# ucas-vg/PointTinyBenchmark

Measured on NVIDIA H100. Metric: cpr_head_refine_img_per_s_1333x800, higher is better.
Workload: dtype fp32

## Files before the change

include/ptb_b200.h:

```cpp
#ifndef PTB_B200_H_
#define PTB_B200_H_

#include <stdint.h>

#ifdef __cplusplus
extern "C" {
#endif

#define PTB_ABI_VERSION 1

int ptb_abi_version(void);
const char* ptb_last_error(void);
uint64_t ptb_launch_count(void);
int ptb_reset_stream_state(void* stream);

int ptb_cpr_bag_gather(const float* map, int B, int H, int W, int C, int ld,
                       const float* centers , const int32_t* bag_img , int G,
                       const float* offsets , int K, float stride,
                       float reach_px ,
                       const int32_t* pad_hw ,
                       float* out_feats , float* out_pts , uint8_t* out_valid ,
                       void* stream);

int ptb_cpr_bag_gather_bwd(const float* grad_out , int B, int H, int W, int C, int ld,
// ... 217 lines not shown
                            int B, int H, int W, int Cin, float* y , double* gn_stats, void* stream);
int ptb_gn_relu_apply(const float* y, const double* gn_stats, const float* gamma, const float* beta, int B, int HW, int C,
                      int groups, float eps, int relu, float* out_hi, float* out_lo, void* stream);
int ptb_split_f16(const float* x, int64_t n, int auto_scale, void* hi, void* lo, float* dev_inv_scale, void* workspace, void* stream);
int ptb_conv3x3_pack_weight_f16(const float* w_oihw, int Cout, int Cin, float scale, void* w_h, void* w_l, void* stream);
int ptb_conv3x3_c256_f16x2(const void* x_h, const void* x_l, const void* w_h, const void* w_l, int B, int H, int W, int Cin,
                           float out_scale, const float* dev_out_scale, float* y, double* gn_stats, void* stream);
int ptb_conv_tc_pack_weight_f16(const float* w , int n_out, int n_mma, int Cin, int taps, float scale,
                                void* w_h, void* w_l, void* stream);
int ptb_conv_tc_f16x2(const void* x_h, const void* x_l, const void* w_h, const void* w_l, int B, int H, int W, int Cin, int taps,
                      int n_out, int n_mma, float out_scale, const float* dev_out_scale, const float* bias, float* y, int ldy,
                      void* stream);
int ptb_gn_relu_apply_f16(const float* y, const double* gn_stats, const float* gamma, const float* beta, int B, int HW, int C,
                          int groups, float eps, int relu, void* out_h, void* out_l, int* overflow_flag, void* stream);
#define PTB_DTYPE_F16 1
#define PTB_DTYPE_BF16 2
int ptb_split_f16_from_bf16(const void* x, int64_t n, void* hi, void* lo, float* dev_inv_scale, void* workspace, void* stream);
int ptb_conv_tc_f16x1a(const void* x_h, const void* w_h, const void* w_l, int B, int H, int W, int Cin, int taps, int n_out, int n_mma,
                       float out_scale, const float* dev_out_scale, const float* bias, float* y, int ldy, double* gn_stats ,
                       void* stream);
int ptb_conv_tc_f16x2_half_out(const void* x_h, const void* x_l, const void* w_h, const void* w_l, int B, int H, int W, int Cin, int taps,
                               int n_out, int n_mma, float out_scale, const float* dev_out_scale, const float* bias, void* y, int y_dtype,
                               int ldy, void* stream);

uint64_t ptb_max_iou_assign_workspace(int N, int n_gt);
int ptb_max_iou_assign(const float* bboxes, int N, const float* gt_bboxes, int n_gt, const int32_t* gt_labels ,
                       const float* gt_bboxes_ignore , int n_ignore, float pos_iou_thr, float neg_iou_lo, float neg_iou_hi,
                       float min_pos_iou, int gt_max_assign_all, int match_low_quality, float ignore_iof_thr, int ignore_wrt_candidates,
                       int64_t* out_gt_inds, float* out_max_overlaps, int64_t* out_labels, void* workspace, uint64_t workspace_bytes,
                       void* stream);
int ptb_bbox_overlaps(const float* boxes1, int m, const float* boxes2, int n, int mode_iof, float* out , void* stream);

uint64_t ptb_gn_relu_bwd_workspace(int B, int HW, int C, int groups);
int ptb_gn_relu_bwd(const float* da, const float* y, const double* gn_stats, const float* gamma, const float* beta, int B, int HW, int C,
                    int groups, float eps, int relu, void* workspace, float* dy, float* dgamma ,
                    float* dbeta , unsigned int* amax_bits , void* stream);
int ptb_split_f16_amax(const float* x, int64_t n, const unsigned int* dev_amax_bits, void* hi, void* lo, float* dev_inv_scale,
                       void* stream);
uint64_t ptb_conv3x3_wgrad_workspace(int B, int H, int W);
int ptb_conv3x3_wgrad_f16x2(const void* dy_h, const void* dy_l, const void* x_h, const void* x_l, int B, int H, int W, int Cout, int Cin,
                            float scale, const float* dev_scale_dy , const float* dev_scale_x , void* workspace,
                            float* dw , int accumulate, void* stream);

uint64_t ptb_conv_tc_wgrad_workspace(int B, int H, int W, int taps);
int ptb_conv_tc_wgrad_f16x2(const void* dy_h, const void* dy_l , const void* x_h, const void* x_l ,
                            int B, int H, int W, int Cout, int Cin, int taps, float scale, const float* dev_scale_dy,
// ... 10 lines not shown
```

pointtinybenchmark_b200/_lib.py:

```python
import ctypes
import os

_HERE = os.path.dirname(os.path.abspath(__file__))
LIB_PATH = os.path.join(_HERE, 'libptb_b200.so')

_lib = None
MISSING = []

c_int, c_float, c_void_p, c_u64, c_i64 = ctypes.c_int, ctypes.c_float, ctypes.c_void_p, ctypes.c_uint64, ctypes.c_int64


class RefineCfg(ctypes.Structure):
    _fields_ = [('merge_th', c_float), ('gt_alpha', c_float), ('refine_th', c_float), ('flags', ctypes.c_int32)]


class MatchCost(ctypes.Structure):
    _fields_ = [('kind', ctypes.c_int32), ('weight', c_float), ('alpha', c_float), ('gamma', c_float), ('eps', c_float),
                ('p', ctypes.c_int32), ('norm_with_img_wh', ctypes.c_int32)]


P = c_void_p
SIGNATURES = {
    'ptb_abi_version': (c_int, []),
    'ptb_last_error': (ctypes.c_char_p, []),
# ... 53 lines not shown
    'ptb_hungarian_v2_workspace': (c_u64, [c_int, c_int]),
    'ptb_hungarian_v2_batch': (c_int, [P, P, c_int, c_int, c_int, c_int, P, P, P, P, P]),
    'ptb_point_assigner': (c_int, [P, c_int, P, c_int, c_float, c_int, P, P, c_u64, P]),
    'ptb_point_assigner_workspace': (c_u64, [c_int, c_int]),
    'ptb_sigmoid_focal_fwd_bwd': (c_int, [P, P, P, c_i64, c_int, c_float, c_float, P, P, P, P]),
    'ptb_smooth_l1_fwd_bwd': (c_int, [P, P, P, c_i64, c_float, c_float, P, P, P, P]),
    'ptb_sigmoid_bce_fwd_bwd': (c_int, [P, P, P, c_i64, c_int, P, P, P, P]),
    'ptb_mse_fwd_bwd': (c_int, [P, P, P, c_i64, c_float, P, P, P, P]),
    'ptb_sigmoid_bce_cw_fwd_bwd': (c_int, [P, P, P, P, c_i64, c_int, P, P, P, P]),
    'ptb_softmax_ce_fwd_bwd': (c_int, [P, P, P, P, c_i64, c_int, P, P, P, P]),
    'ptb_split_tf32': (c_int, [P, c_i64, P, P, P]),
    'ptb_conv3x3_pack_weight': (c_int, [P, c_int, c_int, P, P, P]),
    'ptb_conv3x3_c256_tf32x3': (c_int, [P, P, P, P, c_int, c_int, c_int, c_int, P, P, P]),
    'ptb_gn_relu_apply': (c_int, [P, P, P, P, c_int, c_int, c_int, c_int, c_float, c_int, P, P, P]),
    'ptb_split_f16': (c_int, [P, c_i64, c_int, P, P, P, P, P]),
    'ptb_conv3x3_pack_weight_f16': (c_int, [P, c_int, c_int, c_float, P, P, P]),
    'ptb_conv3x3_c256_f16x2': (c_int, [P, P, P, P, c_int, c_int, c_int, c_int, c_float, P, P, P, P]),
    'ptb_conv_tc_pack_weight_f16': (c_int, [P, c_int, c_int, c_int, c_int, c_float, P, P, P]),
    'ptb_conv_tc_f16x2': (c_int, [P, P, P, P, c_int, c_int, c_int, c_int, c_int, c_int, c_int, c_float, P, P, P, c_int, P]),
    'ptb_gn_relu_apply_f16': (c_int, [P, P, P, P, c_int, c_int, c_int, c_int, c_float, c_int, P, P, P, P]),
    'ptb_split_f16_from_bf16': (c_int, [P, c_i64, P, P, P, P, P]),
    'ptb_conv_tc_f16x1a': (c_int, [P, P, P, c_int, c_int, c_int, c_int, c_int, c_int, c_int, c_float, P, P, P, c_int, P, P]),
    'ptb_conv_tc_f16x2_half_out': (c_int, [P, P, P, P, c_int, c_int, c_int, c_int, c_int, c_int, c_int, c_float, P, P, P, c_int, c_int, P]),
    'ptb_max_iou_assign_workspace': (c_u64, [c_int, c_int]),
    'ptb_max_iou_assign': (c_int, [P, c_int, P, c_int, P, P, c_int, c_float, c_float, c_float, c_float, c_int, c_int, c_float, c_int,
                                   P, P, P, P, c_u64, P]),
    'ptb_bbox_overlaps': (c_int, [P, c_int, P, c_int, c_int, P, P]),
    'ptb_gn_relu_bwd_workspace': (c_u64, [c_int, c_int, c_int, c_int]),
    'ptb_gn_relu_bwd': (c_int, [P, P, P, P, P, c_int, c_int, c_int, c_int, c_float, c_int, P, P, P, P, P, P]),
    'ptb_split_f16_amax': (c_int, [P, c_i64, P, P, P, P, P]),
    'ptb_conv3x3_wgrad_workspace': (c_u64, [c_int, c_int, c_int]),
    'ptb_conv3x3_wgrad_f16x2': (c_int, [P, P, P, P, c_int, c_int, c_int, c_int, c_int, c_float, P, P, P, P, c_int, P]),
    'ptb_conv_tc_wgrad_workspace': (c_u64, [c_int, c_int, c_int, c_int]),
    'ptb_conv_tc_wgrad_f16x2': (c_int, [P, P, P, P, c_int, c_int, c_int, c_int, c_int, c_int, c_float, P, P, P, P, c_int, P]),
    'ptb_col_sum_workspace': (c_u64, [c_i64, c_int]),
    'ptb_col_sum': (c_int, [P, c_i64, c_int, c_int, P, P, P]),
}


def load():
    global _lib
    if _lib is not None:
        return _lib
    if not os.path.exists(LIB_PATH):
        raise RuntimeError(
            f'{LIB_PATH} is missing: build it with `python -c "import __graft_entry__ as g; g.build()"` '
# ... 24 lines not shown
```

pointtinybenchmark_b200/csrc/conv_tc.cu:

```cuda
#include "tc_ptx.cuh"
#include <cuda_bf16.h>
#include <stdlib.h>
#include <type_traits>

namespace ptb {

constexpr int CV_N = 256;
constexpr int CV_N_MAX = 512;
constexpr int CV_BM = 128;
constexpr int CV_NT = 128;
constexpr int CV_KB = 16;
constexpr int CV_KB_F16 = 32;
constexpr int CV_KH = 3;
constexpr int CV_A_STAGES = 4;
constexpr int CV_B_STAGES = 8;
constexpr uint32_t CV_A_BYTES = (CV_BM + 2 * 32) * 64;
constexpr uint32_t CV_B_BYTES = CV_NT * 64;
constexpr uint32_t CV_A_STAGE_BYTES = 2 * CV_A_BYTES;
constexpr uint32_t CV_B_STAGE_BYTES = 2 * CV_B_BYTES;
constexpr uint32_t CV_RING_BYTES = CV_A_STAGES * CV_A_STAGE_BYTES + CV_B_STAGES * CV_B_STAGE_BYTES;
constexpr uint32_t CV_SMEM_BYTES = CV_RING_BYTES + 1024  + 256 ;
static_assert(CV_SMEM_BYTES <= 227 * 1024, "the conv rings must fit the 227 KB of opt-in shared memory");
static_assert(2 * 8 * (CV_A_STAGES + CV_B_STAGES) <= 256, "the conv barriers must fit their 256 B");
constexpr int CV_THREADS = 384;

struct ConvShape {
  int B, H, W, Cin;
  int tiles_h, tiles_w;
  int n_main, n_right, n_bottom, per_img, n_tiles;
  int right_w0, right_h;
  int bottom_h0;
  int n_slices;
  int taps;
  int n_out;
  int ldy;
};

struct ConvMaps {
  CUtensorMap x[3][2];
  CUtensorMap w[2];
};
struct TileAt {
  int b, h0, w0, shape, twl;
};
__device__ __forceinline__ TileAt tile_at(const ConvShape& cs, int tile) {
  TileAt t;
  t.b = tile / cs.per_img;
  const int r = tile - t.b * cs.per_img;
  if (r < cs.n_main) {
    t.shape = 0; t.twl = 4; t.h0 = (r / cs.tiles_w) * 8; t.w0 = (r % cs.tiles_w) * 16;
  } else if (r < cs.n_main + cs.n_right) {
    t.shape = 2; t.twl = 3; t.h0 = (r - cs.n_main) * 16; t.w0 = cs.right_w0;
  } else {
    t.shape = 1; t.twl = 5; t.h0 = cs.bottom_h0; t.w0 = (r - cs.n_main - cs.n_right) * 32;
  }
  return t;
}

template <bool F16, int NT, bool A_LO_ZERO = false, typename OutT = float>
__global__ void __launch_bounds__(CV_THREADS, 1)
conv_tc_kernel(const __grid_constant__ ConvMaps mp, ConvShape cs, OutT* __restrict__ y, double* __restrict__ stats ,
               float out_scale, const float* __restrict__ dev_out_scale, const float* __restrict__ bias) {
  static_assert(F16 || NT == 128, "the TF32 mode runs 128-channel slices");
  static_assert(F16 || (!A_LO_ZERO && std::is_same<OutT, float>::value), "half-precision inputs and outputs belong to the fp16 mode");
  constexpr int KBC = F16 ? CV_KB_F16 : CV_KB;
  extern __shared__ uint8_t smem_raw[];
  const uint32_t smem_base = (smem_u32(smem_raw) + 1023u) & ~1023u;
  const uint32_t sA_base = smem_base, sB_base = smem_base + CV_A_STAGES * CV_A_STAGE_BYTES;
  const uint32_t bar_base = smem_base + CV_RING_BYTES;
  auto full_a = [&](int s) { return bar_base + 8u * s; };
  auto empty_a = [&](int s) { return bar_base + 8u * (CV_A_STAGES + s); };
  auto full_b = [&](int s) { return bar_base + 8u * (2 * CV_A_STAGES + s); };
  auto empty_b = [&](int s) { return bar_base + 8u * (2 * CV_A_STAGES + CV_B_STAGES + s); };

  const int wg = threadIdx.x >> 7;
  const int kblocks_per_tap = cs.Cin / KBC;
  const int n_kh = cs.taps == 9 ? CV_KH : 1;
  const int n_boxes_item = (cs.taps / n_kh) * kblocks_per_tap;
  const int n_items = cs.n_tiles * cs.n_slices;

  if (threadIdx.x == 0) {
    for (int s = 0; s < CV_A_STAGES; ++s) {
      mbar_init(full_a(s), 1);
      mbar_init(empty_a(s), 8);
    }
    for (int s = 0; s < CV_B_STAGES; ++s) {
      mbar_init(full_b(s), 1);
      mbar_init(empty_b(s), 8);
    }
    asm volatile("fence.mbarrier_init.release.cluster;" ::: "memory");
  }
  __syncthreads();

  if (wg == 0) {
    regs_dealloc<40>();
    if (threadIdx.x == 0) {
      int a_st = 0, b_st = 0;
      uint32_t a_ph = 0, b_ph = 0;
      for (int item = blockIdx.x; item < n_items; item += gridDim.x) {
        const int tile = item / cs.n_slices, n0 = (item - tile * cs.n_slices) * NT;
        const TileAt ta = tile_at(cs, tile);
        const uint32_t a_bytes = (uint32_t)(CV_BM + ((n_kh - 1) << ta.twl)) * 64u;
        for (int ks = 0; ks < n_boxes_item; ++ks) {
          const int kw = cs.taps == 9 ? ks / kblocks_per_tap : 1, cblk = ks - (ks / kblocks_per_tap) * kblocks_per_tap;
          mbar_wait(empty_a(a_st), a_ph ^ 1u);
          const uint32_t sA_hi = sA_base + a_st * CV_A_STAGE_BYTES;
          mbar_expect_tx(full_a(a_st), (A_LO_ZERO ? 1 : 2) * a_bytes);
          const int aw = ta.w0 + kw - 1, ah = ta.h0 - (n_kh > 1 ? 1 : 0);
          tma_load_4d(&mp.x[ta.shape][0], full_a(a_st), sA_hi, cblk * KBC, aw, ah, ta.b);
          if constexpr (!A_LO_ZERO) tma_load_4d(&mp.x[ta.shape][1], full_a(a_st), sA_hi + CV_A_BYTES, cblk * KBC, aw, ah, ta.b);
          if (++a_st == CV_A_STAGES) { a_st = 0; a_ph ^= 1u; }
          for (int kh = 0; kh < n_kh; ++kh) {
            const int tap = cs.taps == 9 ? 3 * kh + kw : 0;
            const int kcol = tap * cs.Cin + cblk * KBC;
            mbar_wait(empty_b(b_st), b_ph ^ 1u);
            const uint32_t sB_hi = sB_base + b_st * CV_B_STAGE_BYTES;
            mbar_expect_tx(full_b(b_st), 2 * NT * 64);
            tma_load_2d(&mp.w[0], full_b(b_st), sB_hi, kcol, n0);
            tma_load_2d(&mp.w[1], full_b(b_st), sB_hi + CV_B_BYTES, kcol, n0);
            if (++b_st == CV_B_STAGES) { b_st = 0; b_ph ^= 1u; }
          }
        }
      }
    }
  } else {
    regs_alloc<232>();
    const int cw = wg - 1;
    const int t = threadIdx.x & 127, warp = t >> 5, lane = t & 31;
    const float sc = F16 ? (dev_out_scale ? __fmul_rn(out_scale, *dev_out_scale) : out_scale) : 1.f;
    float acc[NT / 2], cor[NT / 2];
    int a_st = 0, b_st = 0;
    uint32_t a_ph = 0, b_ph = 0;
    for (int item = blockIdx.x; item < n_items; item += gridDim.x) {
      const int tile = item / cs.n_slices, n0 = (item - tile * cs.n_slices) * NT;
      const TileAt ta = tile_at(cs, tile);
      const uint32_t kh_step = 64u << ta.twl;
      auto k_loop = [&](auto kh_n_) {
        constexpr int KH_N = decltype(kh_n_)::value;
        int prev_a = 0, prev_b = 0;
        for (int ks = 0; ks < n_boxes_item; ++ks) {
          mbar_wait(full_a(a_st), a_ph);
          const uint32_t sA_hi = sA_base + a_st * CV_A_STAGE_BYTES + (uint32_t)cw * (CV_BM * 64 / 2);
          const uint32_t sA_lo = sA_hi + CV_A_BYTES;
#pragma unroll
          for (int kh = 0; kh < KH_N; ++kh) {
            mbar_wait(full_b(b_st), b_ph);
            const uint32_t a_off = kh_step * kh, sB_hi = sB_base + b_st * CV_B_STAGE_BYTES, sB_lo = sB_hi + CV_B_BYTES;
            wgmma_fence();
#pragma unroll
// ... 75 lines not shown
            ss = fmaf(v0, v0, ss);
            ss = fmaf(v1, v1, ss);
          }
        }
        if constexpr (NT == 128) { part[2 * i] = s; part[2 * i + 1] = ss; }
      }
      if constexpr (NT == 128) {
        if (stats) {
          auto level = [&](auto o_) {
            constexpr int o = decltype(o_)::value;
            const bool up = (lane & o) != 0;
#pragma unroll
            for (int i = 0; i < o; ++i) {
              const float send = up ? part[i] : part[i + o];
              const float recv = __shfl_xor_sync(0xffffffffu, send, o);
              part[i] = (up ? part[i + o] : part[i]) + recv;
            }
          };
          level(std::integral_constant<int, 16>{}); level(std::integral_constant<int, 8>{}); level(std::integral_constant<int, 4>{});
          level(std::integral_constant<int, 2>{}); level(std::integral_constant<int, 1>{});
          atomicAdd(stats + ((size_t)ta.b * 32 + (n0 >> 3) + (lane >> 1)) * 2 + (lane & 1), (double)part[0]);
        }
      }
    }
  }
}

__device__ __forceinline__ float tf32_hi(float x) { return __uint_as_float(__float_as_uint(x) & 0xFFFFE000u); }

__global__ void __launch_bounds__(256)
split_tf32_kernel(const float4* __restrict__ x, long long n4, float4* __restrict__ hi, float4* __restrict__ lo) {
  for (long long i = (long long)blockIdx.x * 256 + threadIdx.x; i < n4; i += (long long)gridDim.x * 256) {
    const float4 v = __ldcs(x + i);
    float4 h = make_float4(tf32_hi(v.x), tf32_hi(v.y), tf32_hi(v.z), tf32_hi(v.w));
    hi[i] = h;
    lo[i] = make_float4(v.x - h.x, v.y - h.y, v.z - h.z, v.w - h.w);
  }
}

__global__ void __launch_bounds__(256)
gn_relu_apply_kernel(const float4* __restrict__ y, const double* __restrict__ stats, const float* __restrict__ gamma,
                     const float* __restrict__ beta, int HW, int C, int groups, float eps, int relu, long long n4,
                     float4* __restrict__ out_hi, float4* __restrict__ out_lo) {
  const int c4n = C >> 2;
  const int cpg = C / groups;
  const double inv_n = 1.0 / ((double)HW * cpg);
// ... 309 lines not shown
  if (n == 0) return 0;
  long long blocks = (n / 4 + 255) / 256;
  const long long cap = (long long)sm_count() * 16;
  if (blocks > cap) blocks = cap;
  split_tf32_kernel<<<(unsigned)blocks, 256, 0, (cudaStream_t)stream>>>(reinterpret_cast<const float4*>(x), n / 4,
                                                                       reinterpret_cast<float4*>(hi), reinterpret_cast<float4*>(lo));
  return check_launch("ptb_split_tf32");
}

extern "C" int ptb_conv3x3_pack_weight(const float* w_oihw, int Cout, int Cin, float* w_hi, float* w_lo, void* stream) {
  PTB_REQUIRE(Cout > 0 && Cin > 0 && w_oihw && w_hi && w_lo, "shape / NULL");
  const long long n = (long long)Cout * Cin * 9;
  pack_conv_weight_kernel<<<(unsigned)((n + 255) / 256), 256, 0, (cudaStream_t)stream>>>(w_oihw, Cout, Cin, w_hi, w_lo);
  return check_launch("ptb_conv3x3_pack_weight");
}

template <bool F16, int NT, bool A_LO_ZERO = false, typename OutT = float>
static int conv_launch_nt(const ConvMaps& mp, const ConvShape& cs, OutT* y, double* gn_stats, float out_scale, const float* dev_out_scale,
                          const float* bias, void* stream) {
  if (cudaFuncSetAttribute(conv_tc_kernel<F16, NT, A_LO_ZERO, OutT>, cudaFuncAttributeMaxDynamicSharedMemorySize, (int)CV_SMEM_BYTES) != cudaSuccess)
    return fail("%s", "cudaFuncSetAttribute(MaxDynamicSharedMemorySize) failed for the conv kernel");
  int grid = sm_count();
  if (grid > cs.n_tiles * cs.n_slices) grid = cs.n_tiles * cs.n_slices;
  conv_tc_kernel<F16, NT, A_LO_ZERO, OutT><<<grid, CV_THREADS, CV_SMEM_BYTES, (cudaStream_t)stream>>>(mp, cs, y, gn_stats, out_scale, dev_out_scale, bias);
  return 0;
}

template <bool F16, bool A_LO_ZERO = false, typename OutT = float>
static int conv_launch(const void* x_hi, const void* x_lo, const void* w_hi, const void* w_lo, int B, int H, int W, int Cin, int taps,
                       int n_out, int n_mma, OutT* y, int ldy, const float* bias, double* gn_stats, float out_scale,
                       const float* dev_out_scale, void* stream, const char* what) {
  ConvShape cs;
  cs.B = B; cs.H = H; cs.W = W; cs.Cin = Cin;
  {
    const int rh = H % 8, rw = W % 16;
    const bool bottom = rh >= 1 && rh <= 4;
    cs.tiles_h = bottom ? H / 8 : (H + 7) / 8;
    cs.bottom_h0 = cs.tiles_h * 8;
    cs.n_bottom = bottom ? (W + 31) / 32 : 0;
    const bool right = rw >= 1 && rw <= 8 && cs.tiles_h > 0;
    cs.tiles_w = right ? W / 16 : (W + 15) / 16;
    cs.right_w0 = cs.tiles_w * 16;
    cs.right_h = cs.tiles_h * 8 < H ? cs.tiles_h * 8 : H;
    cs.n_right = right ? (cs.right_h + 15) / 16 : 0;
    cs.n_main = cs.tiles_h * cs.tiles_w;
    cs.per_img = cs.n_main + cs.n_right + cs.n_bottom;
    cs.n_tiles = B * cs.per_img;
  }
  const int nt = (!F16 || n_mma > 64) ? CV_NT : n_mma > 32 ? 64 : n_mma > 16 ? 32 : 16;
  PTB_REQUIRE(!gn_stats || (n_out == CV_N && n_mma == CV_N && nt == CV_NT), "GroupNorm statistics need 256 output channels (32 groups of 8)");
  cs.n_slices = (n_mma + nt - 1) / nt;
  cs.taps = taps; cs.n_out = n_out; cs.ldy = ldy;
  ConvMaps mp;
  int rc;
  for (int sh = 0; sh < 3; ++sh) {
    if ((rc = make_act_map(&mp.x[sh][0], x_hi, B, H, W, Cin, F16, sh, taps == 9 ? 2 : 0))) return rc;
    if (A_LO_ZERO) mp.x[sh][1] = mp.x[sh][0];
    else if ((rc = make_act_map(&mp.x[sh][1], x_lo, B, H, W, Cin, F16, sh, taps == 9 ? 2 : 0))) return rc;
  }
  if ((rc = make_w_map(&mp.w[0], w_hi, n_mma, taps * Cin, F16, nt))) return rc;
  if ((rc = make_w_map(&mp.w[1], w_lo, n_mma, taps * Cin, F16, nt))) return rc;
  if constexpr (!F16) rc = conv_launch_nt<false, 128>(mp, cs, y, gn_stats, out_scale, dev_out_scale, bias, stream);
  else if (nt == 128) rc = conv_launch_nt<true, 128, A_LO_ZERO, OutT>(mp, cs, y, gn_stats, out_scale, dev_out_scale, bias, stream);
  else if constexpr (!std::is_same<OutT, float>::value) return fail("%s: a half-precision output needs more than 64 output channels", what);
  else if (nt == 64) rc = conv_launch_nt<true, 64, A_LO_ZERO>(mp, cs, y, gn_stats, out_scale, dev_out_scale, bias, stream);
  else if (nt == 32) rc = conv_launch_nt<true, 32, A_LO_ZERO>(mp, cs, y, gn_stats, out_scale, dev_out_scale, bias, stream);
  else rc = conv_launch_nt<true, 16, A_LO_ZERO>(mp, cs, y, gn_stats, out_scale, dev_out_scale, bias, stream);
  if (rc) return rc;
  return check_launch(what);
}

extern "C" int ptb_conv3x3_c256_tf32x3(const float* x_hi, const float* x_lo, const float* w_hi, const float* w_lo, int B, int H,
                                       int W, int Cin, float* y, double* gn_stats, void* stream) {
  PTB_REQUIRE(B > 0 && H > 0 && W > 0 && Cin > 0, "shape");
  PTB_REQUIRE(Cin % CV_KB == 0, "Cin must be a multiple of 16");
  PTB_REQUIRE(x_hi && x_lo && w_hi && w_lo && y, "NULL input");
  PTB_REQUIRE(((uintptr_t)x_hi % 16 == 0) && ((uintptr_t)x_lo % 16 == 0) && ((uintptr_t)w_hi % 16 == 0) &&
                  ((uintptr_t)w_lo % 16 == 0) && ((uintptr_t)y % 16 == 0), "16-byte alignment");
  return conv_launch<false>(x_hi, x_lo, w_hi, w_lo, B, H, W, Cin, 9, CV_N, CV_N, y, CV_N, nullptr, gn_stats, 1.f, nullptr, stream,
                            "ptb_conv3x3_c256_tf32x3");
}

extern "C" int ptb_conv3x3_c256_f16x2(const void* x_h, const void* x_l, const void* w_h, const void* w_l, int B, int H, int W, int Cin,
                                      float out_scale, const float* dev_out_scale, float* y, double* gn_stats, void* stream) {
// ... 75 lines not shown
  PTB_REQUIRE(((uintptr_t)x_h % 16 == 0) && ((uintptr_t)x_l % 16 == 0) && ((uintptr_t)w_h % 16 == 0) && ((uintptr_t)w_l % 16 == 0) &&
                  ((uintptr_t)y % 16 == 0), "16-byte alignment");
  return conv_launch<true>(x_h, x_l, w_h, w_l, B, H, W, Cin, taps, n_out, n_mma, y, ldy, bias, nullptr, out_scale, dev_out_scale, stream,
                           "ptb_conv_tc_f16x2");
}

static int conv_tc_check_shape(int B, int H, int W, int Cin, int taps, int n_out, int n_mma, int ldy) {
  PTB_REQUIRE(B > 0 && H > 0 && W > 0 && Cin > 0 && (taps == 1 || taps == 9), "shape");
  PTB_REQUIRE(Cin % CV_KB_F16 == 0, "Cin must be a multiple of 32");
  PTB_REQUIRE(n_out > 0 && n_mma >= n_out && n_mma % 16 == 0 && n_mma <= CV_N_MAX, "n_mma must be a multiple of 16 in [n_out, 512]");
  PTB_REQUIRE(ldy >= n_out && ldy % 4 == 0, "ldy must be a multiple of 4 and >= n_out");
  return 0;
}

extern "C" int ptb_conv_tc_f16x1a(const void* x_h, const void* w_h, const void* w_l, int B, int H, int W, int Cin, int taps, int n_out,
                                  int n_mma, float out_scale, const float* dev_out_scale, const float* bias, float* y, int ldy,
                                  double* gn_stats, void* stream) {
  if (int rc = conv_tc_check_shape(B, H, W, Cin, taps, n_out, n_mma, ldy)) return rc;
  PTB_REQUIRE(x_h && w_h && w_l && y, "NULL input");
  PTB_REQUIRE(((uintptr_t)x_h % 16 == 0) && ((uintptr_t)w_h % 16 == 0) && ((uintptr_t)w_l % 16 == 0) && ((uintptr_t)y % 16 == 0),
              "16-byte alignment");
  return conv_launch<true, true>(x_h, nullptr, w_h, w_l, B, H, W, Cin, taps, n_out, n_mma, y, ldy, bias, gn_stats, out_scale, dev_out_scale,
                                 stream, "ptb_conv_tc_f16x1a");
}

extern "C" int ptb_conv_tc_f16x2_half_out(const void* x_h, const void* x_l, const void* w_h, const void* w_l, int B, int H, int W, int Cin,
                                          int taps, int n_out, int n_mma, float out_scale, const float* dev_out_scale, const float* bias,
                                          void* y, int y_dtype, int ldy, void* stream) {
  if (int rc = conv_tc_check_shape(B, H, W, Cin, taps, n_out, n_mma, ldy)) return rc;
  PTB_REQUIRE(y_dtype == PTB_DTYPE_F16 || y_dtype == PTB_DTYPE_BF16, "y_dtype must be PTB_DTYPE_F16 or PTB_DTYPE_BF16");
  PTB_REQUIRE(x_h && x_l && w_h && w_l && y, "NULL input");
  PTB_REQUIRE(((uintptr_t)x_h % 16 == 0) && ((uintptr_t)x_l % 16 == 0) && ((uintptr_t)w_h % 16 == 0) && ((uintptr_t)w_l % 16 == 0) &&
                  ((uintptr_t)y % 16 == 0), "16-byte alignment");
  if (y_dtype == PTB_DTYPE_F16)
    return conv_launch<true, false, __half>(x_h, x_l, w_h, w_l, B, H, W, Cin, taps, n_out, n_mma, reinterpret_cast<__half*>(y), ldy, bias,
                                            nullptr, out_scale, dev_out_scale, stream, "ptb_conv_tc_f16x2_half_out");
  return conv_launch<true, false, __nv_bfloat16>(x_h, x_l, w_h, w_l, B, H, W, Cin, taps, n_out, n_mma, reinterpret_cast<__nv_bfloat16*>(y),
                                                 ldy, bias, nullptr, out_scale, dev_out_scale, stream, "ptb_conv_tc_f16x2_half_out");
}

extern "C" int ptb_split_f16_from_bf16(const void* x, int64_t n, void* hi, void* lo, float* dev_inv_scale, void* workspace, void* stream) {
  PTB_REQUIRE(n >= 0 && n % 8 == 0, "n must be a multiple of 8");
  PTB_REQUIRE(((uintptr_t)x % 16 == 0) && ((uintptr_t)hi % 16 == 0) && ((uintptr_t)lo % 16 == 0), "16-byte alignment");
  PTB_REQUIRE(workspace && dev_inv_scale, "a 4-byte workspace and dev_inv_scale are required");
  if (n == 0) return 0;
  cudaStream_t st = (cudaStream_t)stream;
// ... 58 lines not shown
```

pointtinybenchmark_b200/layers.py:

```python
import math

import torch
import torch.nn as nn
import torch.nn.functional as F


class ConvModule(nn.Module):

    def __init__(self, cin, cout, k=3, stride=1, padding=1, norm_cfg=None, bias='auto', act=True):
        super().__init__()
        with_norm = norm_cfg is not None
        if bias == 'auto':
            bias = not with_norm
        self.conv = nn.Conv2d(cin, cout, k, stride, padding, bias=bias)
        self.norm_name = None
        if with_norm:
            t = norm_cfg['type']
            if t == 'GN':
                self.norm_name = 'gn'
                self.add_module('gn', nn.GroupNorm(norm_cfg['num_groups'], cout))
            elif t in ('BN', 'SyncBN'):
                self.norm_name = 'bn'
                self.add_module('bn', nn.BatchNorm2d(cout))
            else:
# ... 140 lines not shown
        c = m.conv
        if not (c.in_channels == 256 and c.out_channels == 256 and c.kernel_size == (3, 3) and c.stride == (1, 1)
                and c.padding == (1, 1) and c.dilation == (1, 1) and c.groups == 1 and c.bias is None and m.norm_name == 'gn'
                and m.with_act and m.gn.num_groups == 32 and m.gn.affine):
            return False
    return True


class _TowerTCFn(torch.autograd.Function):

    @staticmethod
    def forward(ctx, xm, convs, *params):
        from . import ops
        n_layers = len(convs)
        groups, eps = [m.gn.num_groups for m in convs], [float(m.gn.eps) for m in convs]
        h, l, dev_inv = _first_operands(xm)
        half_in = xm.dtype != torch.float32
        flag = torch.zeros(1, dtype=torch.int32, device=xm.device)
        saved, out = [], None
        for i in range(n_layers):
            gamma, beta = params[3 * i + 1], params[3 * i + 2]
            wh, wl, inv_w = _packed_weight_f16(convs[i])
            inv_x = dev_inv if i == 0 else None
            y, stats = ops.conv3x3_c256_f16(h, l, wh, wl, inv_w, inv_x)
            saved += [xm, None, y, stats] if i == 0 and half_in else [h, l, y, stats]
            if i == n_layers - 1:
                out = ops.gn_relu_apply(y, stats, gamma.detach(), beta.detach(), groups[i], eps[i], True, split=False)
            else:
                h, l = ops.gn_relu_apply_f16(y, stats, gamma.detach(), beta.detach(), groups[i], eps[i], True, flag)
        ctx.n_layers, ctx.groups, ctx.eps, ctx.convs = n_layers, groups, eps, convs
        ctx.dev_inv, ctx.in_dtype = dev_inv, xm.dtype
        ctx.save_for_backward(*saved, *[p.detach() for p in params])
        return out

    @staticmethod
    def backward(ctx, dout):
        from . import ops
        n = ctx.n_layers
        saved = ctx.saved_tensors
        acts, params = saved[:4 * n], saved[4 * n:]
        da = dout.contiguous()
        grads = [None] * (3 * n)
        for i in reversed(range(n)):
            h, l, y, stats = acts[4 * i:4 * i + 4]
            inv_x = ctx.dev_inv if i == 0 else None
            if i == 0 and ctx.in_dtype != torch.float32:
                h, l, inv_x = _first_operands(h)
                if l is None:
                    l = torch.zeros_like(h)
            w, gamma, beta = params[3 * i], params[3 * i + 1], params[3 * i + 2]
            dy, dg, db, amax = ops.gn_relu_bwd(da, y, stats, gamma, beta, ctx.groups[i], ctx.eps[i], True)
            dyh, dyl, inv_dy = ops.split_f16_amax(dy, amax)
# ... 4 lines not shown
                da = ops.conv_tc_f16(dyh, dyl, _packed_weight_f16_t(ctx.convs[i]), 9, w.shape[1], dev_out_scale=inv_dy,
                                     out_dtype=ctx.in_dtype if i == 0 else torch.float32)
            else:
                da = None
        return (da, None, *grads)


def tower(convs, x, info=None, want='fp32'):
    import os
    mode = os.environ.get('PTB_CONV_MODE', 'f16x2')
    if x.dtype in HALF_INPUT_DTYPES and not x.is_cuda:
        raise RuntimeError(f'tower: expected a CUDA tensor for a {x.dtype} input (pointtinybenchmark_b200 has no CPU path)')
    plan = input_plan(x.dtype, mode)
    if want == 'f16pair' and not (_tc_supported(convs, x) and mode == 'f16x2' and all(m.conv.in_channels % 32 == 0 for m in convs)):
        return None
    if _tc_supported(convs, x) and mode == 'f16x2' and all(m.conv.in_channels % 32 == 0 for m in convs):
        from . import ops
        xm = ops.to_nhwc(x).contiguous()
        h, l, dev_inv = _first_operands(xm)
        flag = torch.zeros(1, dtype=torch.int32, device=x.device)
        out = None
        for i, m in enumerate(convs):
            wh, wl, inv_w = _packed_weight_f16(m)
            y, stats = ops.conv3x3_c256_f16(h, l, wh, wl, inv_w, dev_inv if i == 0 else None)
            if i == len(convs) - 1 and want == 'fp32':
                out = ops.gn_relu_apply(y, stats, m.gn.weight.detach(), m.gn.bias.detach(), m.gn.num_groups, m.gn.eps, True, split=False)
            else:
                h, l = ops.gn_relu_apply_f16(y, stats, m.gn.weight.detach(), m.gn.bias.detach(), m.gn.num_groups, m.gn.eps, True, flag)
        if info is not None:
            info['backend'] = 'wgmma-f16x2'
            info['input_path'] = plan[0]
            info['overflow_flag'] = flag
        if want == 'f16pair':
            return h, l
        return out.permute(0, 3, 1, 2)
    if _tc_supported(convs, x):
        from . import ops
        xm = ops.to_nhwc(x).contiguous()
        hi, lo = ops.split_tf32(xm)
        out = None
        for i, m in enumerate(convs):
            wh, wl = _packed_weight(m)
            y, stats = ops.conv3x3_c256(hi, lo, wh, wl)
            last = i == len(convs) - 1
            res = ops.gn_relu_apply(y, stats, m.gn.weight.detach(), m.gn.bias.detach(), m.gn.num_groups, m.gn.eps, True,
                                    split=not last)
            if last:
                out = res
            else:
                hi, lo = res
        if info is not None:
# ... 25 lines not shown
```

pointtinybenchmark_b200/ops.py:

```python
import ctypes
import math

import torch

from . import _lib
from ._lib import RefineCfg, check


def _ptr(t):
    return ctypes.c_void_p(t.data_ptr()) if t is not None else ctypes.c_void_p(0)


def _stream():
    return ctypes.c_void_p(torch.cuda.current_stream().cuda_stream)


def _chk(t, dtype, name):
    if not isinstance(t, torch.Tensor) or not t.is_cuda:
        raise RuntimeError(f'{name}: expected a CUDA tensor (pointtinybenchmark_b200 has no CPU path)')
    if t.dtype != dtype:
        raise TypeError(f'{name}: expected {dtype}, got {t.dtype}')
    if not t.is_contiguous():
        raise ValueError(f'{name}: must be contiguous')
    return t
# ... 781 lines not shown
    l = torch.empty_like(h)
    check(lib.ptb_conv3x3_pack_weight_f16(_ptr(w), Cout, Cin, float(scale), _ptr(h), _ptr(l), _stream()), 'ptb_conv3x3_pack_weight_f16')
    return h, l, 1.0 / scale


def conv3x3_c256_f16(x_h, x_l, w_h, w_l, out_scale, dev_out_scale=None, want_stats=True):
    lib = _lib.load()
    _chk(x_h, torch.float16, 'x_h'); _chk(w_h, torch.float16, 'w_h'); _chk(w_l, torch.float16, 'w_l')
    B, H, W, Cin = x_h.shape
    if w_h.shape != (256, 9 * Cin):
        raise ValueError('packed weight must be (256, 9*Cin)')
    y = torch.empty((B, H, W, 256), dtype=torch.float32, device=x_h.device)
    stats = torch.zeros((B, 32, 2), dtype=torch.float64, device=x_h.device) if want_stats else None
    if x_l is None:
        check(lib.ptb_conv_tc_f16x1a(_ptr(x_h), _ptr(w_h), _ptr(w_l), B, H, W, Cin, 9, 256, 256, float(out_scale), _ptr(dev_out_scale), None,
                                     _ptr(y), 256, _ptr(stats), _stream()), 'ptb_conv_tc_f16x1a')
        return y, stats
    _chk(x_l, torch.float16, 'x_l')
    check(lib.ptb_conv3x3_c256_f16x2(_ptr(x_h), _ptr(x_l), _ptr(w_h), _ptr(w_l), B, H, W, Cin, float(out_scale), _ptr(dev_out_scale),
                                     _ptr(y), _ptr(stats), _stream()), 'ptb_conv3x3_c256_f16x2')
    return y, stats


def gn_relu_apply_f16(y, stats, gamma, beta, groups=32, eps=1e-5, relu=True, overflow_flag=None):
    lib = _lib.load()
    _chk(y, torch.float32, 'y'); _chk(stats, torch.float64, 'stats')
    B, H, W, C = y.shape
    h = torch.empty(y.shape, dtype=torch.float16, device=y.device)
    l = torch.empty_like(h)
    check(lib.ptb_gn_relu_apply_f16(_ptr(y), _ptr(stats), _ptr(gamma), _ptr(beta), B, H * W, C, groups, float(eps), 1 if relu else 0,
                                    _ptr(h), _ptr(l), _ptr(overflow_flag), _stream()), 'ptb_gn_relu_apply_f16')
    return h, l


def gn_relu_bwd(da, y, stats, gamma, beta, groups=32, eps=1e-5, relu=True, want_amax=True):
    lib = _lib.load()
    _chk(da, torch.float32, 'da'); _chk(y, torch.float32, 'y'); _chk(stats, torch.float64, 'stats')
    B, H, W, C = y.shape
    dev = y.device
    nbytes = int(lib.ptb_gn_relu_bwd_workspace(B, H * W, C, groups))
    if nbytes == 0:
        raise ValueError(f'ptb_gn_relu_bwd: unsupported shape C={C}, groups={groups}')
    ws = torch.empty(nbytes, dtype=torch.uint8, device=dev)
    dy = torch.empty_like(y)
    dg = torch.empty(C, dtype=torch.float32, device=dev)
    db = torch.empty(C, dtype=torch.float32, device=dev)
# ... 93 lines not shown
```

Measured before the change: 2298.

## Fuse GroupNorm+ReLU apply into persistent conv kernel via cross-block image completion counters

Adds a cooperative-launched variant of the wgmma conv kernel in which producer-warpgroup spare warps (and, after the MMA loop, all warps) apply GroupNorm+ReLU. Per-image completion counters published with release/acquire atomics let each image be normalised as soon as all of its tiles and statistics are done, overlapping the apply with later images' convolution. This removes a separate apply kernel launch and overlaps its memory traffic with compute. In exchange it lowers the consumer register budget, adds spin-waits, and relies on cooperative residency, falling back to the unfused path if that is not available.

```diff
diff --git a/include/ptb_b200.h b/include/ptb_b200.h
--- a/include/ptb_b200.h
+++ b/include/ptb_b200.h
@@ -263,6 +263,9 @@
 int ptb_conv_tc_f16x2_half_out(const void* x_h, const void* x_l, const void* w_h, const void* w_l, int B, int H, int W, int Cin, int taps,
                                int n_out, int n_mma, float out_scale, const float* dev_out_scale, const float* bias, void* y, int y_dtype,
                                int ldy, void* stream);
+int ptb_conv3x3_c256_f16_gn(const void* x_h, const void* x_l , const void* w_h, const void* w_l, int B, int H, int W, int Cin,
+                            float out_scale, const float* dev_out_scale, float* y, void* workspace, const float* gamma, const float* beta,
+                            float eps, void* out, void* out_l , int* overflow_flag , void* stream);
 
 uint64_t ptb_max_iou_assign_workspace(int N, int n_gt);
 int ptb_max_iou_assign(const float* bboxes, int N, const float* gt_bboxes, int n_gt, const int32_t* gt_labels ,
diff --git a/pointtinybenchmark_b200/_lib.py b/pointtinybenchmark_b200/_lib.py
--- a/pointtinybenchmark_b200/_lib.py
+++ b/pointtinybenchmark_b200/_lib.py
@@ -99,6 +99,7 @@
     'ptb_split_f16_from_bf16': (c_int, [P, c_i64, P, P, P, P, P]),
     'ptb_conv_tc_f16x1a': (c_int, [P, P, P, c_int, c_int, c_int, c_int, c_int, c_int, c_int, c_float, P, P, P, c_int, P, P]),
     'ptb_conv_tc_f16x2_half_out': (c_int, [P, P, P, P, c_int, c_int, c_int, c_int, c_int, c_int, c_int, c_float, P, P, P, c_int, c_int, P]),
+    'ptb_conv3x3_c256_f16_gn': (c_int, [P, P, P, P, c_int, c_int, c_int, c_int, c_float, P, P, P, P, P, c_float, P, P, P, P]),
     'ptb_max_iou_assign_workspace': (c_u64, [c_int, c_int]),
     'ptb_max_iou_assign': (c_int, [P, c_int, P, c_int, P, P, c_int, c_float, c_float, c_float, c_float, c_int, c_int, c_float, c_int,
                                    P, P, P, P, c_u64, P]),
diff --git a/pointtinybenchmark_b200/csrc/conv_tc.cu b/pointtinybenchmark_b200/csrc/conv_tc.cu
--- a/pointtinybenchmark_b200/csrc/conv_tc.cu
+++ b/pointtinybenchmark_b200/csrc/conv_tc.cu
@@ -21,7 +21,7 @@
 constexpr uint32_t CV_RING_BYTES = CV_A_STAGES * CV_A_STAGE_BYTES + CV_B_STAGES * CV_B_STAGE_BYTES;
 constexpr uint32_t CV_SMEM_BYTES = CV_RING_BYTES + 1024  + 256 ;
 static_assert(CV_SMEM_BYTES <= 227 * 1024, "the conv rings must fit the 227 KB of opt-in shared memory");
-static_assert(2 * 8 * (CV_A_STAGES + CV_B_STAGES) <= 256, "the conv barriers must fit their 256 B");
+static_assert(2 * 8 * (CV_A_STAGES + CV_B_STAGES) + 8 <= 256, "the conv barriers and the item counter must fit their 256 B");
 constexpr int CV_THREADS = 384;
 
 struct ConvShape {
@@ -57,12 +57,124 @@
   return t;
 }
 
-template <bool F16, int NT, bool A_LO_ZERO = false, typename OutT = float>
+constexpr int CV_GN_NONE = 0, CV_GN_F16 = 1, CV_GN_F32 = 2;
+constexpr int CV_APPLY_WARPS = 3;
+constexpr int CV_MMA_WARPS = 8;
+struct GnFuse {
+  const float* gamma;
+  const float* beta;
+  float eps;
+  void* out;
+  __half* out_l;
+  int* overflow_flag;
+  int* done;
+};
+constexpr uint32_t CV_CNT_OFFSET = 2 * 8 * (CV_A_STAGES + CV_B_STAGES);
+
+__device__ __forceinline__ int ld_acquire_gpu(const int* p) {
+  int v;
+  asm volatile("ld.acquire.gpu.global.b32 %0, [%1];" : "=r"(v) : "l"(p) : "memory");
+  return v;
+}
+__device__ __forceinline__ void red_release_gpu_add(int* p, int v) {
+  asm volatile("red.release.gpu.global.add.s32 [%0], %1;" ::"l"(p), "r"(v) : "memory");
+}
+__device__ __forceinline__ int ld_acquire_cta_shared(uint32_t a) {
+  int v;
+  asm volatile("ld.acquire.cta.shared::cta.b32 %0, [%1];" : "=r"(v) : "r"(a) : "memory");
+  return v;
+}
+__device__ __forceinline__ void red_release_cta_shared_add(uint32_t a, int v) {
+  asm volatile("red.release.cta.shared::cta.add.s32 [%0], %1;" ::"r"(a), "r"(v) : "memory");
+}
+__device__ __forceinline__ void wait_count(const int* p, int target, int lane) {
+  if (lane == 0) {
+    uint32_t ns = 32, polls = 0;
+    while (ld_acquire_gpu(p) < target) {
+      __nanosleep(ns);
+      if (ns < 1024) ns <<= 1;
+      if (++polls > (1u << 24)) __trap();
+    }
+  }
+  __syncwarp();
+}
+__device__ __forceinline__ void publish_image(uint32_t cnt, int* done_b, int item, int last, int lane) {
+  if (lane == 0) {
+    const int n = (last - item) / (int)gridDim.x + 1;
+    const int through = (item - (int)blockIdx.x) / (int)gridDim.x + n;
+    uint32_t ns = 32, polls = 0;
+    while (ld_acquire_cta_shared(cnt) < through * (CV_MMA_WARPS / 2) || ld_acquire_cta_shared(cnt + 4) < through * (CV_MMA_WARPS / 2)) {
+      __nanosleep(ns);
+      if (ns < 1024) ns <<= 1;
+      if (++polls > (1u << 24)) __trap();
+    }
+    red_release_gpu_add(done_b, n * CV_MMA_WARPS);
+  }
+  __syncwarp();
+}
+
+template <int GN>
+__device__ __forceinline__ void gn_apply_item(const ConvShape& cs, const GnFuse& gf, const float* __restrict__ y,
+                                              const double* __restrict__ stats, int item, int member, int team, int lane,
+                                              bool& clamped) {
+  const int tile = item / cs.n_slices, n0 = (item - tile * cs.n_slices) * CV_NT;
+  const TileAt ta = tile_at(cs, tile);
+  const int c = n0 + 4 * lane, g = c >> 3;
+  const int HW = cs.H * cs.W, cpg = CV_N / 32;
+  const double inv_n = 1.0 / ((double)HW * cpg);
+  const double s = __ldcg(stats + ((size_t)ta.b * 32 + g) * 2), ss = __ldcg(stats + ((size_t)ta.b * 32 + g) * 2 + 1);
+  const double mean = s * inv_n;
+  double var = ss * inv_n - mean * mean;
+  var = var < 0.0 ? 0.0 : var;
+  const float rstd = (float)(1.0 / sqrt(var + (double)gf.eps));
+  const float mu = (float)mean;
+  const float4 ga = __ldg(reinterpret_cast<const float4*>(gf.gamma + c)), be = __ldg(reinterpret_cast<const float4*>(gf.beta + c));
+  const int h_end = ta.shape == 2 ? cs.right_h : cs.H;
+  const int tw_mask = (1 << ta.twl) - 1;
+  const size_t img = (size_t)ta.b * HW * CV_N + c;
+  const float* __restrict__ yb = y + img;
+  constexpr int U = 4;
+  for (int p0 = member; p0 < CV_BM; p0 += U * team) {
+    float4 v[U];
+    int at[U];
+#pragma unroll
+    for (int u = 0; u < U; ++u) {
+      const int p = p0 + u * team;
+      const int h = ta.h0 + (p >> ta.twl), w = ta.w0 + (p & tw_mask);
+      at[u] = p < CV_BM && h < h_end && w < cs.W ? (h * cs.W + w) * CV_N : -1;
+      if (at[u] >= 0) v[u] = __ldcg(reinterpret_cast<const float4*>(yb + at[u]));
+    }
+#pragma unroll
+    for (int u = 0; u < U; ++u) {
+      if (at[u] < 0) continue;
+      float o[4] = {v[u].x, v[u].y, v[u].z, v[u].w};
+      o[0] = fmaf((o[0] - mu) * rstd, ga.x, be.x); o[1] = fmaf((o[1] - mu) * rstd, ga.y, be.y);
+      o[2] = fmaf((o[2] - mu) * rstd, ga.z, be.z); o[3] = fmaf((o[3] - mu) * rstd, ga.w, be.w);
+#pragma unroll
+      for (int j = 0; j < 4; ++j) o[j] = fmaxf(o[j], 0.f);
+      if constexpr (GN == CV_GN_F16) {
+        __align__(8) __half h[4], l[4];
+#pragma unroll
+        for (int j = 0; j < 4; ++j) {
+          if (fabsf(o[j]) > 60000.f) { o[j] = copysignf(60000.f, o[j]); clamped = true; }
+          split_h2(o[j], h[j], l[j]);
+        }
+        *reinterpret_cast<uint2*>(reinterpret_cast<__half*>(gf.out) + img + at[u]) = *reinterpret_cast<uint2*>(h);
+        *reinterpret_cast<uint2*>(gf.out_l + img + at[u]) = *reinterpret_cast<uint2*>(l);
+      } else {
+        *reinterpret_cast<float4*>(reinterpret_cast<float*>(gf.out) + img + at[u]) = make_float4(o[0], o[1], o[2], o[3]);
+      }
+    }
+  }
+}
+
+template <bool F16, int NT, bool A_LO_ZERO = false, typename OutT = float, int GN = CV_GN_NONE>
 __global__ void __launch_bounds__(CV_THREADS, 1)
 conv_tc_kernel(const __grid_constant__ ConvMaps mp, ConvShape cs, OutT* __restrict__ y, double* __restrict__ stats ,
-               float out_scale, const float* __restrict__ dev_out_scale, const float* __restrict__ bias) {
+               float out_scale, const float* __restrict__ dev_out_scale, const float* __restrict__ bias, GnFuse gf) {
   static_assert(F16 || NT == 128, "the TF32 mode runs 128-channel slices");
   static_assert(F16 || (!A_LO_ZERO && std::is_same<OutT, float>::value), "half-precision inputs and outputs belong to the fp16 mode");
+  static_assert(GN == CV_GN_NONE || (F16 && NT == 128 && std::is_same<OutT, float>::value), "the fused GroupNorm apply runs on fp32 y, NT 128");
   constexpr int KBC = F16 ? CV_KB_F16 : CV_KB;
   extern __shared__ uint8_t smem_raw[];
   const uint32_t smem_base = (smem_u32(smem_raw) + 1023u) & ~1023u;
@@ -88,12 +200,31 @@
       mbar_init(full_b(s), 1);
       mbar_init(empty_b(s), 8);
     }
+    if constexpr (GN != CV_GN_NONE) asm volatile("st.shared.v2.u32 [%0], {0, 0};" ::"r"(bar_base + CV_CNT_OFFSET) : "memory");
     asm volatile("fence.mbarrier_init.release.cluster;" ::: "memory");
   }
   __syncthreads();
 
   if (wg == 0) {
-    regs_dealloc<40>();
+    if constexpr (GN != CV_GN_NONE) {
+      regs_dealloc<72>();
+      const int warp = threadIdx.x >> 5, lane = threadIdx.x & 31;
+      if (warp >= 1) {
+        const int items_per_img = cs.per_img * cs.n_slices;
+        bool clamped = false;
+        for (int item = blockIdx.x; item < n_items; item += gridDim.x) {
+          const int b = item / items_per_img;
+          if (b == cs.B - 1) break;
+          if (warp == 1 && item - (int)gridDim.x < b * items_per_img)
+            publish_image(bar_base + CV_CNT_OFFSET, gf.done + b, item, (b + 1) * items_per_img - 1, lane);
+          wait_count(gf.done + b, items_per_img * CV_MMA_WARPS, lane);
+          gn_apply_item<GN>(cs, gf, y, stats, item, warp - 1, CV_APPLY_WARPS, lane, clamped);
+        }
+        if (clamped && gf.overflow_flag) *gf.overflow_flag = 1;
+      }
+    } else {
+      regs_dealloc<40>();
+    }
     if (threadIdx.x == 0) {
       int a_st = 0, b_st = 0;
       uint32_t a_ph = 0, b_ph = 0;
@@ -124,7 +255,8 @@
       }
     }
   } else {
-    regs_alloc<232>();
+    if constexpr (GN != CV_GN_NONE) regs_alloc<216>();
+    else regs_alloc<232>();
     const int cw = wg - 1;
     const int t = threadIdx.x & 127, warp = t >> 5, lane = t & 31;
     const float sc = F16 ? (dev_out_scale ? __fmul_rn(out_scale, *dev_out_scale) : out_scale) : 1.f;
@@ -246,6 +378,25 @@
           atomicAdd(stats + ((size_t)ta.b * 32 + (n0 >> 3) + (lane >> 1)) * 2 + (lane & 1), (double)part[0]);
         }
       }
+      if constexpr (GN != CV_GN_NONE) {
+        __syncwarp();
+        if (lane == 0) red_release_cta_shared_add(bar_base + CV_CNT_OFFSET + 4u * cw, 1);
+      }
+    }
+  }
+  if constexpr (GN != CV_GN_NONE) {
+    const int warp = threadIdx.x >> 5, lane = threadIdx.x & 31;
+    if (warp >= 1) {
+      const int items_per_img = cs.per_img * cs.n_slices, last0 = (cs.B - 1) * items_per_img;
+      bool clamped = false;
+      int item = (int)blockIdx.x;
+      if (item < last0) item += (last0 - item + (int)gridDim.x - 1) / (int)gridDim.x * (int)gridDim.x;
+      if (warp == 1 && item < n_items) publish_image(bar_base + CV_CNT_OFFSET, gf.done + cs.B - 1, item, n_items - 1, lane);
+      for (; item < n_items; item += gridDim.x) {
+        wait_count(gf.done + cs.B - 1, items_per_img * CV_MMA_WARPS, lane);
+        gn_apply_item<GN>(cs, gf, y, stats, item, warp - 1, CV_APPLY_WARPS + CV_MMA_WARPS, lane, clamped);
+      }
+      if (clamped && gf.overflow_flag) *gf.overflow_flag = 1;
     }
   }
 }
@@ -601,15 +752,48 @@
     return fail("%s", "cudaFuncSetAttribute(MaxDynamicSharedMemorySize) failed for the conv kernel");
   int grid = sm_count();
   if (grid > cs.n_tiles * cs.n_slices) grid = cs.n_tiles * cs.n_slices;
-  conv_tc_kernel<F16, NT, A_LO_ZERO, OutT><<<grid, CV_THREADS, CV_SMEM_BYTES, (cudaStream_t)stream>>>(mp, cs, y, gn_stats, out_scale, dev_out_scale, bias);
+  conv_tc_kernel<F16, NT, A_LO_ZERO, OutT><<<grid, CV_THREADS, CV_SMEM_BYTES, (cudaStream_t)stream>>>(mp, cs, y, gn_stats, out_scale, dev_out_scale, bias,
+                                                                                                    GnFuse{});
   return 0;
 }
 
-template <bool F16, bool A_LO_ZERO = false, typename OutT = float>
-static int conv_launch(const void* x_hi, const void* x_lo, const void* w_hi, const void* w_lo, int B, int H, int W, int Cin, int taps,
-                       int n_out, int n_mma, OutT* y, int ldy, const float* bias, double* gn_stats, float out_scale,
-                       const float* dev_out_scale, void* stream, const char* what) {
-  ConvShape cs;
+template <bool A_LO_ZERO, int GN>
+static int conv_gn_launch(const ConvMaps& mp, const ConvShape& cs, float* y, double* stats, float out_scale, const float* dev_out_scale,
+                          const GnFuse& gf, cudaStream_t st, bool* launched) {
+  *launched = false;
+  auto kern = conv_tc_kernel<true, CV_NT, A_LO_ZERO, float, GN>;
+  if (cudaFuncSetAttribute(kern, cudaFuncAttributeMaxDynamicSharedMemorySize, (int)CV_SMEM_BYTES) != cudaSuccess)
+    return fail("%s", "cudaFuncSetAttribute(MaxDynamicSharedMemorySize) failed for the fused conv kernel");
+  const int n_items = cs.n_tiles * cs.n_slices;
+  const int grid = sm_count() < n_items ? sm_count() : n_items;
+  int per_sm = 0;
+  if (cudaOccupancyMaxActiveBlocksPerMultiprocessor(&per_sm, kern, CV_THREADS, CV_SMEM_BYTES) != cudaSuccess) {
+    (void)cudaGetLastError();
+    return 0;
+  }
+  if (per_sm * sm_count() < grid) return 0;
+  cudaLaunchConfig_t cfg = {};
+  cfg.gridDim = dim3((unsigned)grid);
+  cfg.blockDim = dim3(CV_THREADS);
+  cfg.dynamicSmemBytes = CV_SMEM_BYTES;
+  cfg.stream = st;
+  cudaLaunchAttribute attr[1];
+  attr[0].id = cudaLaunchAttributeCooperative;
+  attr[0].val.cooperative = 1;
+  cfg.attrs = attr;
+  cfg.numAttrs = 1;
+  const float* no_bias = nullptr;
+  if (cudaLaunchKernelEx(&cfg, kern, mp, cs, y, stats, out_scale, dev_out_scale, no_bias, gf) != cudaSuccess) {
+    (void)cudaGetLastError();
+    return 0;
+  }
+  *launched = true;
+  return 0;
+}
+
+template <bool F16, bool A_LO_ZERO>
+static int conv_prepare(ConvShape& cs, ConvMaps& mp, int* nt_out, const void* x_hi, const void* x_lo, const void* w_hi, const void* w_lo,
+                        int B, int H, int W, int Cin, int taps, int n_out, int n_mma, int ldy, const double* gn_stats) {
   cs.B = B; cs.H = H; cs.W = W; cs.Cin = Cin;
   {
     const int rh = H % 8, rw = W % 16;
@@ -630,7 +814,6 @@
   PTB_REQUIRE(!gn_stats || (n_out == CV_N && n_mma == CV_N && nt == CV_NT), "GroupNorm statistics need 256 output channels (32 groups of 8)");
   cs.n_slices = (n_mma + nt - 1) / nt;
   cs.taps = taps; cs.n_out = n_out; cs.ldy = ldy;
-  ConvMaps mp;
   int rc;
   for (int sh = 0; sh < 3; ++sh) {
     if ((rc = make_act_map(&mp.x[sh][0], x_hi, B, H, W, Cin, F16, sh, taps == 9 ? 2 : 0))) return rc;
@@ -639,6 +822,19 @@
   }
   if ((rc = make_w_map(&mp.w[0], w_hi, n_mma, taps * Cin, F16, nt))) return rc;
   if ((rc = make_w_map(&mp.w[1], w_lo, n_mma, taps * Cin, F16, nt))) return rc;
+  *nt_out = nt;
+  return 0;
+}
+
+template <bool F16, bool A_LO_ZERO = false, typename OutT = float>
+static int conv_launch(const void* x_hi, const void* x_lo, const void* w_hi, const void* w_lo, int B, int H, int W, int Cin, int taps,
+                       int n_out, int n_mma, OutT* y, int ldy, const float* bias, double* gn_stats, float out_scale,
+                       const float* dev_out_scale, void* stream, const char* what) {
+  ConvShape cs;
+  ConvMaps mp;
+  int nt = 0;
+  int rc = conv_prepare<F16, A_LO_ZERO>(cs, mp, &nt, x_hi, x_lo, w_hi, w_lo, B, H, W, Cin, taps, n_out, n_mma, ldy, gn_stats);
+  if (rc) return rc;
   if constexpr (!F16) rc = conv_launch_nt<false, 128>(mp, cs, y, gn_stats, out_scale, dev_out_scale, bias, stream);
   else if (nt == 128) rc = conv_launch_nt<true, 128, A_LO_ZERO, OutT>(mp, cs, y, gn_stats, out_scale, dev_out_scale, bias, stream);
   else if constexpr (!std::is_same<OutT, float>::value) return fail("%s: a half-precision output needs more than 64 output channels", what);
@@ -760,6 +956,45 @@
               "16-byte alignment");
   return conv_launch<true, true>(x_h, nullptr, w_h, w_l, B, H, W, Cin, taps, n_out, n_mma, y, ldy, bias, gn_stats, out_scale, dev_out_scale,
                                  stream, "ptb_conv_tc_f16x1a");
+}
+
+extern "C" int ptb_conv3x3_c256_f16_gn(const void* x_h, const void* x_l, const void* w_h, const void* w_l, int B, int H, int W, int Cin,
+                                       float out_scale, const float* dev_out_scale, float* y, void* workspace, const float* gamma,
+                                       const float* beta, float eps, void* out, void* out_l, int* overflow_flag, void* stream) {
+  PTB_REQUIRE(B > 0 && H > 0 && W > 0 && Cin > 0, "shape");
+  PTB_REQUIRE(Cin % CV_KB_F16 == 0, "Cin must be a multiple of 32");
+  PTB_REQUIRE(x_h && w_h && w_l && y && workspace && gamma && beta && out, "NULL input");
+  PTB_REQUIRE(((uintptr_t)x_h % 16 == 0) && ((uintptr_t)x_l % 16 == 0) && ((uintptr_t)w_h % 16 == 0) && ((uintptr_t)w_l % 16 == 0) &&
+                  ((uintptr_t)y % 16 == 0) && ((uintptr_t)workspace % 8 == 0) && ((uintptr_t)gamma % 16 == 0) && ((uintptr_t)beta % 16 == 0) &&
+                  ((uintptr_t)out % 16 == 0) && ((uintptr_t)out_l % 16 == 0), "alignment");
+  cudaStream_t st = (cudaStream_t)stream;
+  double* stats = reinterpret_cast<double*>(workspace);
+  GnFuse gf;
+  gf.gamma = gamma; gf.beta = beta; gf.eps = eps; gf.out = out; gf.out_l = reinterpret_cast<__half*>(out_l);
+  gf.overflow_flag = overflow_flag;
+  gf.done = reinterpret_cast<int*>(stats + (size_t)B * 32 * 2);
+  ConvShape cs;
+  ConvMaps mp;
+  int nt = 0, rc;
+  bool launched = false;
+  if (x_l) {
+    if ((rc = conv_prepare<true, false>(cs, mp, &nt, x_h, x_l, w_h, w_l, B, H, W, Cin, 9, CV_N, CV_N, CV_N, stats))) return rc;
+    rc = out_l ? conv_gn_launch<false, CV_GN_F16>(mp, cs, y, stats, out_scale, dev_out_scale, gf, st, &launched)
+               : conv_gn_launch<false, CV_GN_F32>(mp, cs, y, stats, out_scale, dev_out_scale, gf, st, &launched);
+  } else {
+    if ((rc = conv_prepare<true, true>(cs, mp, &nt, x_h, nullptr, w_h, w_l, B, H, W, Cin, 9, CV_N, CV_N, CV_N, stats))) return rc;
+    rc = out_l ? conv_gn_launch<true, CV_GN_F16>(mp, cs, y, stats, out_scale, dev_out_scale, gf, st, &launched)
+               : conv_gn_launch<true, CV_GN_F32>(mp, cs, y, stats, out_scale, dev_out_scale, gf, st, &launched);
+  }
+  if (rc) return rc;
+  if (launched) return check_launch("ptb_conv3x3_c256_f16_gn");
+  if (x_l) rc = conv_launch<true>(x_h, x_l, w_h, w_l, B, H, W, Cin, 9, CV_N, CV_N, y, CV_N, nullptr, stats, out_scale, dev_out_scale, stream,
+                                  "ptb_conv3x3_c256_f16_gn/conv");
+  else rc = conv_launch<true, true>(x_h, nullptr, w_h, w_l, B, H, W, Cin, 9, CV_N, CV_N, y, CV_N, nullptr, stats, out_scale, dev_out_scale,
+                                    stream, "ptb_conv3x3_c256_f16_gn/conv");
+  if (rc) return rc;
+  if (out_l) return ptb_gn_relu_apply_f16(y, stats, gamma, beta, B, H * W, CV_N, 32, eps, 1, out, out_l, overflow_flag, stream);
+  return ptb_gn_relu_apply(y, stats, gamma, beta, B, H * W, CV_N, 32, eps, 1, reinterpret_cast<float*>(out), nullptr, stream);
 }
 
 extern "C" int ptb_conv_tc_f16x2_half_out(const void* x_h, const void* x_l, const void* w_h, const void* w_l, int B, int H, int W, int Cin,
diff --git a/pointtinybenchmark_b200/layers.py b/pointtinybenchmark_b200/layers.py
--- a/pointtinybenchmark_b200/layers.py
+++ b/pointtinybenchmark_b200/layers.py
@@ -186,12 +186,14 @@
             gamma, beta = params[3 * i + 1], params[3 * i + 2]
             wh, wl, inv_w = _packed_weight_f16(convs[i])
             inv_x = dev_inv if i == 0 else None
-            y, stats = ops.conv3x3_c256_f16(h, l, wh, wl, inv_w, inv_x)
+            last = i == n_layers - 1
+            a, b, y, stats = ops.conv3x3_c256_f16_gn(h, l, wh, wl, inv_w, inv_x, gamma.detach(), beta.detach(), eps[i], flag,
+                                                     out='fp32' if last else 'f16pair')
             saved += [xm, None, y, stats] if i == 0 and half_in else [h, l, y, stats]
-            if i == n_layers - 1:
-                out = ops.gn_relu_apply(y, stats, gamma.detach(), beta.detach(), groups[i], eps[i], True, split=False)
-            else:
-                h, l = ops.gn_relu_apply_f16(y, stats, gamma.detach(), beta.detach(), groups[i], eps[i], True, flag)
+            if last:
+                out = a
+            else:
+                h, l = a, b
         ctx.n_layers, ctx.groups, ctx.eps, ctx.convs = n_layers, groups, eps, convs
         ctx.dev_inv, ctx.in_dtype = dev_inv, xm.dtype
         ctx.save_for_backward(*saved, *[p.detach() for p in params])
@@ -242,11 +244,13 @@
         out = None
         for i, m in enumerate(convs):
             wh, wl, inv_w = _packed_weight_f16(m)
-            y, stats = ops.conv3x3_c256_f16(h, l, wh, wl, inv_w, dev_inv if i == 0 else None)
-            if i == len(convs) - 1 and want == 'fp32':
-                out = ops.gn_relu_apply(y, stats, m.gn.weight.detach(), m.gn.bias.detach(), m.gn.num_groups, m.gn.eps, True, split=False)
-            else:
-                h, l = ops.gn_relu_apply_f16(y, stats, m.gn.weight.detach(), m.gn.bias.detach(), m.gn.num_groups, m.gn.eps, True, flag)
+            fp32_out = i == len(convs) - 1 and want == 'fp32'
+            a, b, _, _ = ops.conv3x3_c256_f16_gn(h, l, wh, wl, inv_w, dev_inv if i == 0 else None, m.gn.weight.detach(),
+                                                 m.gn.bias.detach(), m.gn.eps, flag, out='fp32' if fp32_out else 'f16pair')
+            if fp32_out:
+                out = a
+            else:
+                h, l = a, b
         if info is not None:
             info['backend'] = 'wgmma-f16x2'
             info['input_path'] = plan[0]
diff --git a/pointtinybenchmark_b200/ops.py b/pointtinybenchmark_b200/ops.py
--- a/pointtinybenchmark_b200/ops.py
+++ b/pointtinybenchmark_b200/ops.py
@@ -827,6 +827,32 @@
     return y, stats
 
 
+def conv3x3_c256_f16_gn(x_h, x_l, w_h, w_l, out_scale, dev_out_scale, gamma, beta, eps=1e-5, overflow_flag=None, out='f16pair'):
+    lib = _lib.load()
+    _chk(x_h, torch.float16, 'x_h'); _chk(w_h, torch.float16, 'w_h'); _chk(w_l, torch.float16, 'w_l')
+    _chk(gamma, torch.float32, 'gamma'); _chk(beta, torch.float32, 'beta')
+    if x_l is not None:
+        _chk(x_l, torch.float16, 'x_l')
+    if out not in ('f16pair', 'fp32'):
+        raise ValueError(f"out must be 'f16pair' or 'fp32', got {out!r}")
+    B, H, W, Cin = x_h.shape
+    if w_h.shape != (256, 9 * Cin) or gamma.shape != (256,) or beta.shape != (256,):
+        raise ValueError('packed weight must be (256, 9*Cin), gamma and beta (256,)')
+    dev = x_h.device
+    y = torch.empty((B, H, W, 256), dtype=torch.float32, device=dev)
+    ws = torch.zeros(B * 64 + (B + 1) // 2, dtype=torch.float64, device=dev)
+    stats = ws[:B * 64].view(B, 32, 2)
+    if out == 'f16pair':
+        a = torch.empty((B, H, W, 256), dtype=torch.float16, device=dev)
+        b = torch.empty_like(a)
+    else:
+        a, b = torch.empty_like(y), None
+    check(lib.ptb_conv3x3_c256_f16_gn(_ptr(x_h), _ptr(x_l), _ptr(w_h), _ptr(w_l), B, H, W, Cin, float(out_scale), _ptr(dev_out_scale),
+                                      _ptr(y), _ptr(ws), _ptr(gamma), _ptr(beta), float(eps), _ptr(a), _ptr(b), _ptr(overflow_flag),
+                                      _stream()), 'ptb_conv3x3_c256_f16_gn')
+    return a, b, y, stats
+
+
 def gn_relu_apply_f16(y, stats, gamma, beta, groups=32, eps=1e-5, relu=True, overflow_flag=None):
     lib = _lib.load()
     _chk(y, torch.float32, 'y'); _chk(stats, torch.float64, 'stats')
```

Result: faster. 2437 (median of 6 runs) (+6.0%).
